# Gilgamesh666666/Point-cloud-registration-based-on-rotation-invariant-feature

Measured on AMD Instinct MI355X. Metric: point-clouds/sec (1024 pts, k=32) PPF+sph-vox forward, higher is better.
Workload: dtype f32; 1 GPU; sph-dg extractor forward: self-KNN k=32 + local PPF + sph-vox r=32^3 + sph-devox + descriptor; clouds_per_gpu=32, points=1024, k=32, resolution=32, channels=64, global_batch=32, parallelism=dp1 (clouds sharded, descriptor all-gather), schedule=6, steps_per_launch=200, distinct_batches=20

## Files before the change

point-cloud-registration-based-on-rotation-invariant-feature_amd/csrc/knn_wsel.hip:

```cpp
#include "knn_spatial.hpp"

namespace pcr {

__device__ inline int pcr_opaque(int v) {
  asm volatile("" : "+v"(v));
  return v;
}

template <int W>
constexpr int wsel_chunk() { return W == 8 ? 2 : 1; }
static inline bool wsel_narrow(int nblk, int b) { return (size_t)nblk * b * 8 > 4096; }
constexpr int kWselCap = 64;
constexpr int kWselTmax = 0x461C3FFF;

#define PCR_WSEL_VCC_STAGE(NAME, CTRL, LOW)                                        \
  __device__ inline unsigned NAME(unsigned x) {                                    \
    unsigned t;                                                                    \
    asm volatile("s_nop 1\n\t"                                                     \
                 "v_sub_co_u32_dpp %1, vcc, %0, %0 " CTRL " row_mask:0xf bank_mask:0xf\n\t" \
                 "s_xor_b32 vcc_lo, vcc_lo, " LOW "\n\t"                           \
                 "s_xor_b32 vcc_hi, vcc_hi, " LOW "\n\t"                           \
                 "v_cndmask_b32_dpp %0, %0, %0, vcc " CTRL " row_mask:0xf bank_mask:0xf" \
                 : "+v"(x), "=&v"(t)                                               \
                 :                                                                 \
                 : "vcc");                                                         \
    return x;                                                                      \
  }
PCR_WSEL_VCC_STAGE(wsel_x1, "quad_perm:[1,0,3,2]", "0x55555555")
PCR_WSEL_VCC_STAGE(wsel_x2, "quad_perm:[2,3,0,1]", "0x33333333")
PCR_WSEL_VCC_STAGE(wsel_m4, "quad_perm:[3,2,1,0]", "0x33333333")
#undef PCR_WSEL_VCC_STAGE
#define PCR_WSEL_MINMAX_STAGE(NAME, LO, HI, MLO, MHI)                              \
  __device__ inline unsigned NAME(unsigned x) {                                    \
    unsigned a;                                                                    \
    asm volatile("s_nop 1\n\t"                                                     \
                 "v_min_u32_dpp %0, %1, %1 " LO " " MLO "\n\t"                     \
                 "v_max_u32_dpp %0, %1, %1 " HI " " MHI                            \
                 : "=&v"(a)                                                        \
                 : "v"(x));                                                        \
    return a;                                                                      \
  }
PCR_WSEL_MINMAX_STAGE(wsel_m8, "row_half_mirror", "row_half_mirror",
                      "row_mask:0xf bank_mask:0x5", "row_mask:0xf bank_mask:0xa")
PCR_WSEL_MINMAX_STAGE(wsel_m16, "row_mirror", "row_mirror",
                      "row_mask:0xf bank_mask:0x3", "row_mask:0xf bank_mask:0xc")
PCR_WSEL_MINMAX_STAGE(wsel_x4, "row_shl:4", "row_shr:4",
                      "row_mask:0xf bank_mask:0x5", "row_mask:0xf bank_mask:0xa")
PCR_WSEL_MINMAX_STAGE(wsel_x8, "row_shl:8", "row_shr:8",
                      "row_mask:0xf bank_mask:0x3", "row_mask:0xf bank_mask:0xc")
#undef PCR_WSEL_MINMAX_STAGE
#define PCR_WSEL_ROW_STAGE(NAME, FETCH, RLO, RHI)                                  \
  __device__ inline unsigned NAME(unsigned x) {                                    \
    unsigned a, p;                                                                 \
    asm volatile("s_nop 1\n\t" FETCH                                               \
                 "s_nop 1\n\t"                                                     \
                 "v_min_u32_dpp %0, %1, %2 quad_perm:[0,1,2,3] row_mask:" RLO " bank_mask:0xf\n\t" \
                 "v_max_u32_dpp %0, %1, %2 quad_perm:[0,1,2,3] row_mask:" RHI " bank_mask:0xf" \
                 : "=&v"(a), "+v"(x), "=&v"(p)                                     \
                 :);                                                               \
    return a;                                                                      \
  }
PCR_WSEL_ROW_STAGE(wsel_x16,
                   "v_mov_b32_e32 %2, %1\n\t"
                   "s_nop 1\n\t"
                   "v_permlane16_swap_b32 %2, %2\n\t",
                   "0x5", "0xa")
PCR_WSEL_ROW_STAGE(wsel_m32,
                   "v_mov_b32_dpp %2, %1 row_mirror row_mask:0xf bank_mask:0xf\n\t"
                   "s_nop 1\n\t"
                   "v_permlane16_swap_b32 %2, %2\n\t",
                   "0x5", "0xa")
PCR_WSEL_ROW_STAGE(wsel_m64,
                   "v_mov_b32_dpp %2, %1 row_mirror row_mask:0xf bank_mask:0xf\n\t"
                   "s_nop 1\n\t"
                   "v_permlane16_swap_b32 %2, %2\n\t"
                   "s_nop 1\n\t"
                   "v_permlane32_swap_b32 %2, %2\n\t",
                   "0x3", "0xc")
#undef PCR_WSEL_ROW_STAGE

__device__ inline unsigned wsel_sort64(unsigned x) {
  x = wsel_x1(x);
  x = wsel_m4(x);
  x = wsel_x1(x);
  x = wsel_m8(x);
  x = wsel_x2(x);
  x = wsel_x1(x);
  x = wsel_m16(x);
  x = wsel_x4(x);
  x = wsel_x2(x);
  x = wsel_x1(x);
  x = wsel_m32(x);
  x = wsel_x8(x);
  x = wsel_x4(x);
  x = wsel_x2(x);
  x = wsel_x1(x);
  x = wsel_m64(x);
  x = wsel_x16(x);
  x = wsel_x8(x);
  x = wsel_x4(x);
  x = wsel_x2(x);
  x = wsel_x1(x);
  asm volatile("s_nop 1");
  return x;
}

__device__ inline unsigned long long wsel_sort64_exact(unsigned long long x, int lane) {
  for (int kk = 2; kk <= 64; kk <<= 1) {
    for (int jj = kk >> 1; jj > 0; jj >>= 1) {
      const int m = jj == (kk >> 1) ? kk - 1 : jj;
      const unsigned long long p = shfl_xor_u64(x, m);
      const bool lower = (lane & jj) == 0;
      x = lower ? (x < p ? x : p) : (x < p ? p : x);
    }
  }
  return x;
}

__device__ inline void wsel_append(unsigned long long m, unsigned addr, unsigned d, int j) {
  unsigned t;
  unsigned long long save;
  asm volatile(
      "s_mov_b64 %1, exec\n\t"
      "s_mov_b64 exec, %2\n\t"
      "v_mbcnt_lo_u32_b32 %0, %3, 0\n\t"
      "v_mbcnt_hi_u32_b32 %0, %4, %0\n\t"
      "v_lshl_add_u32 %0, %0, 2, %5\n\t"
      "ds_write_b32 %0, %6\n\t"
      "ds_write_b32 %0, %7 offset:256\n\t"
      "s_mov_b64 exec, %1"
      : "=&v"(t), "=&s"(save)
      : "s"(m), "s"((unsigned)m), "s"((unsigned)(m >> 32)), "s"(addr), "v"(d), "v"(j)
      : "memory");
}

template <int R, int W>
__global__ __launch_bounds__(W * 64) void knn_wsel_kernel(KnnSet s, int k) {
  constexpr int kWselWaves = W;
  constexpr int kWselChunk = wsel_chunk<W>();
  __shared__ unsigned kbuf_s[kWselWaves][2][kWselCap];
  __shared__ int tile_s[kBlk][kSortedK + 1];
  __shared__ int qnext_s;
  __shared__ int cj_s[R * kBlk];
  static_assert(sizeof(kbuf_s[0][0]) == 256, "wsel_append's offset");
  const int b = blockIdx.y, qblk = blockIdx.x;
  const int wv = __builtin_amdgcn_readfirstlane(threadIdx.x >> 6);
  const int lane = threadIdx.x & 63;
  const size_t cb = (size_t)b * s.npad;
  const int nr = s.npad / kBlk;
  typedef float pf2v __attribute__((ext_vector_type(2)));
  pf2v cx[R / 2], cy[R / 2], cz[R / 2];
  for (int i = threadIdx.x; i < R * kBlk; i += kWselWaves * kBlk)
    cj_s[i] = i < s.npad ? s.j[cb + i] : -1;
#pragma unroll
  for (int h = 0; h < R / 2; h++) {
    float v[2][3];
#pragma unroll
    for (int e = 0; e < 2; e++) {
      const int r = 2 * h + e;
      const bool ok = r < nr;
      const size_t p = cb + (size_t)(ok ? r : nr - 1) * kBlk + lane;
      const float x = s.x[p], y = s.y[p], z = s.z[p];
      v[e][0] = ok ? x : __builtin_nanf("");
      v[e][1] = ok ? y : __builtin_nanf("");
      v[e][2] = ok ? z : __builtin_nanf("");
    }
    cx[h] = pf2v{v[0][0], v[1][0]};
    cy[h] = pf2v{v[0][1], v[1][1]};
    cz[h] = pf2v{v[0][2], v[1][2]};
  }
  const size_t pq = cb + (size_t)qblk * kBlk + lane;
  const float qxl = s.x[pq], qyl = s.y[pq], qzl = s.z[pq];
  const int qjl = s.j[pq];
  if (threadIdx.x == 0) qnext_s = 0;
  __syncthreads();
  auto grab = [&]() {
    int v = 0;
    if (lane == 0)
      v = __hip_atomic_fetch_add(&qnext_s, kWselChunk, __ATOMIC_RELAXED, __HIP_MEMORY_SCOPE_WORKGROUP);
    return v;
  };
  int q0 = __builtin_amdgcn_readfirstlane(grab());
  int tb = kWselTmax;
  if (q0 < kBlk) {
    const float* bx = s.box + ((size_t)b * s.nblk + qblk) * 8;
    const float qx = readlane_f(qxl, q0), qy = readlane_f(qyl, q0), qz = readlane_f(qzl, q0);
    if (min(kBlk, s.n - qblk * kBlk) >= k) {
      const float u = box_ub(qx, qy, qz, bx);
      if (u < PCR_KNN_UNDEF) tb = (int)__float_as_uint(u);
    }
  }
  unsigned* kd = kbuf_s[wv][0];
  int* kj = (int*)kbuf_s[wv][1];
  const unsigned kd_addr =
      (unsigned)(uintptr_t)((__attribute__((address_space(3))) unsigned*)kd);
  const float tgt = 0.5f * (float)(k + kWselCap);
#pragma unroll 1
  for (int qi = q0; qi < kBlk;) {
    const int qj = __builtin_amdgcn_readlane(qjl, qi);
    if (qj < 0) {
      if (lane < kSortedK) tile_s[qi][lane] = 0;
      if (++qi % kWselChunk == 0) qi = __builtin_amdgcn_readfirstlane(grab());
      continue;
    }
    const float qx = readlane_f(qxl, qi), qy = readlane_f(qyl, qi), qz = readlane_f(qzl, qi);
    const pf2v qx2 = {qx, qx}, qy2 = {qy, qy}, qz2 = {qz, qz};
    unsigned db[R];
#pragma unroll
    for (int h = 0; h < R / 2; h++) {
      const pf2v a = qx2 - cx[h], bq = qy2 - cy[h], c = qz2 - cz[h];
      pf2v d = a * a;
      d = __builtin_elementwise_fma(bq, bq, d);
      d = __builtin_elementwise_fma(c, c, d);
      db[2 * h] = __float_as_uint(d[0]);
      db[2 * h + 1] = __float_as_uint(d[1]);
    }
    constexpr bool kKeep = R <= 16;
    unsigned long long msk[kKeep ? R : 1];
    auto count_le = [&](int bits) {
      int pc[4] = {0, 0, 0, 0};
#pragma unroll
      for (int r = 0; r < R; r++) {
        const unsigned long long m = __ballot(db[r] <= (unsigned)bits);
        if (kKeep) msk[kKeep ? r : 0] = m;
        pc[r & 3] += __popcll(m);
      }
      return (pc[0] + pc[1]) + (pc[2] + pc[3]);
    };
    int lo = -1, hi = 0x7F800000, cnt_lo = 0, cnt = 0;
    bool exact = false;
#pragma unroll 1
    for (int pass = 0;; pass++) {
      cnt = count_le(tb);
      if (cnt >= k && cnt <= kWselCap) break;
      if (cnt < k) {
        lo = tb;
        cnt_lo = cnt;
        if (tb >= kWselTmax) break;
      } else {
        hi = tb;
      }
      if (hi - lo <= 1) {
        exact = true;
        break;
      }
      int nb;
      if (pass < 3) {
        const float f = __uint_as_float((unsigned)tb) *
                        __builtin_amdgcn_exp2f(0.6666667f * __builtin_amdgcn_logf(
                                                                tgt * __builtin_amdgcn_rcpf((float)max(cnt, 1))));
        nb = f < 1e30f ? (int)__float_as_uint(f) : kWselTmax;
      } else {
        nb = lo + ((hi - lo) >> 1);
      }
      nb = min(nb, kWselTmax);
      if (nb <= lo || nb >= hi) nb = lo + ((hi - lo) >> 1);
      tb = __builtin_amdgcn_readfirstlane(nb);
    }
    int ntake;
    if (!exact) {
      unsigned addr = kd_addr;
#pragma unroll
      for (int r = 0; r < R; r++) {
        const unsigned long long m = kKeep ? msk[kKeep ? r : 0] : __ballot(db[r] <= (unsigned)tb);
        if (m != 0ull) {
          wsel_append(m, addr, db[r], 64 * r + pcr_opaque(lane));
          addr += 4u * (unsigned)__popcll(m);
        }
      }
      ntake = cnt;
    } else {
      const int need = k - cnt_lo;
      auto cj = [&](int r) { return cj_s[64 * r + lane]; };
      int jl = -1, jh = s.n - 1;
#pragma unroll 1
      while (jh - jl > 1) {
        const int jm = jl + ((jh - jl) >> 1);
        int c = 0;
#pragma unroll
        for (int r = 0; r < R; r++) c += __popcll(__ballot(db[r] == (unsigned)hi && cj(r) <= jm));
        if (c >= need) jh = jm;
        else jl = jm;
      }
      unsigned addr = kd_addr;
#pragma unroll
      for (int r = 0; r < R; r++) {
        const unsigned long long m =
            __ballot(db[r] < (unsigned)hi || (db[r] == (unsigned)hi && cj(r) <= jh));
        if (m != 0ull) {
          wsel_append(m, addr, db[r], 64 * r + pcr_opaque(lane));
          addr += 4u * (unsigned)__popcll(m);
        }
      }
      ntake = k;
    }
    const unsigned dl = lane < ntake ? kd[lane] : 0xFFFFFFFFu;
    unsigned key = lane < ntake ? ((dl >> 6) << 6) | (unsigned)lane : 0x7FFFFFFFu;
    key = wsel_sort64(key);
    const unsigned nxt = (unsigned)__builtin_amdgcn_mov_dpp((int)key, 0x130, 0xF, 0xF, false);
    const bool tie = lane < k && lane + 1 < ntake && (key >> 6) == (nxt >> 6);
    const bool slow = __any(tie);
    if (!slow) {
      const int jo = lane < ntake ? cj_s[kj[key & 63u]] : 0;
      if (lane < k) tile_s[qi][lane] = jo;
    } else {
      unsigned long long skey = ~0ull;
      if (lane < ntake) skey = ((unsigned long long)kd[lane] << 32) | (unsigned)cj_s[kj[lane]];
      skey = wsel_sort64_exact(skey, lane);
      if (lane < k) tile_s[qi][lane] = lane < ntake ? (int)(unsigned)(skey & 0xFFFFFFFFull) : 0;
    }
    __atomic_signal_fence(__ATOMIC_SEQ_CST);
    if (++qi % kWselChunk == 0) qi = __builtin_amdgcn_readfirstlane(grab());
  }
  __syncthreads();
  for (int sl = wv; sl < k; sl += kWselWaves)
    s.sidx[((size_t)b * kSortedK + sl) * s.npad + (size_t)qblk * kBlk + lane] = tile_s[lane][sl];
}

void launch_wsel(const KnnSet& s, int b, int k, hipStream_t st) {
  if (wsel_narrow(s.nblk, b))
    hipLaunchKernelGGL((knn_wsel_kernel<16, 8>), dim3(s.nblk, b), dim3(8 * 64), 0, st, s, k);
  else
    hipLaunchKernelGGL((knn_wsel_kernel<16, 12>), dim3(s.nblk, b), dim3(12 * 64), 0, st, s, k);
}

}
```

Baseline: 462,600 point-clouds/sec.

## Stage cloud coordinates into LDS via DMA and merge append writes

```diff
diff --git a/point-cloud-registration-based-on-rotation-invariant-feature_amd/csrc/knn_wsel.hip b/point-cloud-registration-based-on-rotation-invariant-feature_amd/csrc/knn_wsel.hip
--- a/point-cloud-registration-based-on-rotation-invariant-feature_amd/csrc/knn_wsel.hip
+++ b/point-cloud-registration-based-on-rotation-invariant-feature_amd/csrc/knn_wsel.hip
@@ -1,11 +1,6 @@
 #include "knn_spatial.hpp"
 
 namespace pcr {
-
-__device__ inline int pcr_opaque(int v) {
-  asm volatile("" : "+v"(v));
-  return v;
-}
 
 template <int W>
 constexpr int wsel_chunk() { return W == 8 ? 2 : 1; }
@@ -117,20 +112,22 @@
   return x;
 }
 
-__device__ inline void wsel_append(unsigned long long m, unsigned addr, unsigned d, int j) {
-  unsigned t;
+__device__ __attribute__((always_inline)) inline void wsel_append(unsigned long long m,
+                                                                  unsigned addr, unsigned d,
+                                                                  int lane, int r) {
+  unsigned t, p;
   unsigned long long save;
+  asm volatile("v_add_u32_e32 %0, %2, %1" : "=v"(p) : "v"(lane), "i"(64 * r));
   asm volatile(
       "s_mov_b64 %1, exec\n\t"
       "s_mov_b64 exec, %2\n\t"
       "v_mbcnt_lo_u32_b32 %0, %3, 0\n\t"
       "v_mbcnt_hi_u32_b32 %0, %4, %0\n\t"
       "v_lshl_add_u32 %0, %0, 2, %5\n\t"
-      "ds_write_b32 %0, %6\n\t"
-      "ds_write_b32 %0, %7 offset:256\n\t"
+      "ds_write2st64_b32 %0, %6, %7 offset1:1\n\t"
       "s_mov_b64 exec, %1"
       : "=&v"(t), "=&s"(save)
-      : "s"(m), "s"((unsigned)m), "s"((unsigned)(m >> 32)), "s"(addr), "v"(d), "v"(j)
+      : "s"(m), "s"((unsigned)m), "s"((unsigned)(m >> 32)), "s"(addr), "v"(d), "v"(p)
       : "memory");
 }
 
@@ -141,39 +138,40 @@
   __shared__ unsigned kbuf_s[kWselWaves][2][kWselCap];
   __shared__ int tile_s[kBlk][kSortedK + 1];
   __shared__ int qnext_s;
-  __shared__ int cj_s[R * kBlk];
+  __shared__ __align__(16) float cx_s[R * kBlk], cy_s[R * kBlk], cz_s[R * kBlk];
+  __shared__ __align__(16) int cj_s[R * kBlk];
   static_assert(sizeof(kbuf_s[0][0]) == 256, "wsel_append's offset");
+  static_assert(sizeof(cx_s) % (64 * 16) == 0, "whole LDS-DMA pieces");
   const int b = blockIdx.y, qblk = blockIdx.x;
   const int wv = __builtin_amdgcn_readfirstlane(threadIdx.x >> 6);
   const int lane = threadIdx.x & 63;
   const size_t cb = (size_t)b * s.npad;
-  const int nr = s.npad / kBlk;
+  lds_dma_copy<16>(cx_s, s.x + cb, 4 * s.npad);
+  lds_dma_copy<16>(cy_s, s.y + cb, 4 * s.npad);
+  lds_dma_copy<16>(cz_s, s.z + cb, 4 * s.npad);
+  lds_dma_copy<16>(cj_s, s.j + cb, 4 * s.npad);
+  if (threadIdx.x == 0) qnext_s = 0;
+  wait_vmcnt<0>();
+  __syncthreads();
+  if (s.npad < R * kBlk) {
+    for (int i = s.npad + threadIdx.x; i < R * kBlk; i += kWselWaves * kBlk) {
+      cx_s[i] = cy_s[i] = cz_s[i] = __builtin_nanf("");
+      cj_s[i] = -1;
+    }
+    __syncthreads();
+  }
   typedef float pf2v __attribute__((ext_vector_type(2)));
   pf2v cx[R / 2], cy[R / 2], cz[R / 2];
-  for (int i = threadIdx.x; i < R * kBlk; i += kWselWaves * kBlk)
-    cj_s[i] = i < s.npad ? s.j[cb + i] : -1;
 #pragma unroll
   for (int h = 0; h < R / 2; h++) {
-    float v[2][3];
-#pragma unroll
-    for (int e = 0; e < 2; e++) {
-      const int r = 2 * h + e;
-      const bool ok = r < nr;
-      const size_t p = cb + (size_t)(ok ? r : nr - 1) * kBlk + lane;
-      const float x = s.x[p], y = s.y[p], z = s.z[p];
-      v[e][0] = ok ? x : __builtin_nanf("");
-      v[e][1] = ok ? y : __builtin_nanf("");
-      v[e][2] = ok ? z : __builtin_nanf("");
-    }
-    cx[h] = pf2v{v[0][0], v[1][0]};
-    cy[h] = pf2v{v[0][1], v[1][1]};
-    cz[h] = pf2v{v[0][2], v[1][2]};
-  }
-  const size_t pq = cb + (size_t)qblk * kBlk + lane;
-  const float qxl = s.x[pq], qyl = s.y[pq], qzl = s.z[pq];
-  const int qjl = s.j[pq];
-  if (threadIdx.x == 0) qnext_s = 0;
-  __syncthreads();
+    const int p = 2 * h * kBlk + lane;
+    cx[h] = pf2v{cx_s[p], cx_s[p + kBlk]};
+    cy[h] = pf2v{cy_s[p], cy_s[p + kBlk]};
+    cz[h] = pf2v{cz_s[p], cz_s[p + kBlk]};
+  }
+  const int pq = qblk * kBlk + lane;
+  const float qxl = cx_s[pq], qyl = cy_s[pq], qzl = cz_s[pq];
+  const int qjl = cj_s[pq];
   auto grab = [&]() {
     int v = 0;
     if (lane == 0)
@@ -264,7 +262,7 @@
       for (int r = 0; r < R; r++) {
         const unsigned long long m = kKeep ? msk[kKeep ? r : 0] : __ballot(db[r] <= (unsigned)tb);
         if (m != 0ull) {
-          wsel_append(m, addr, db[r], 64 * r + pcr_opaque(lane));
+          wsel_append(m, addr, db[r], lane, r);
           addr += 4u * (unsigned)__popcll(m);
         }
       }
@@ -288,7 +286,7 @@
         const unsigned long long m =
             __ballot(db[r] < (unsigned)hi || (db[r] == (unsigned)hi && cj(r) <= jh));
         if (m != 0ull) {
-          wsel_append(m, addr, db[r], 64 * r + pcr_opaque(lane));
+          wsel_append(m, addr, db[r], lane, r);
           addr += 4u * (unsigned)__popcll(m);
         }
       }
```

After: 474,700 point-clouds/sec, median of 6. +2.6%, better.
